# lab-cosmo/torch-pme

Hardware: AMD Instinct MI355X
Metric: atom-steps/sec (energy+forces) (higher is better)
Workload: dtype f32

## Files before the change

### torch-pme_amd/csrc/api.hip

```cpp
#include <dlfcn.h>

#include <cmath>
#include <cstring>
#include <map>
#include <string>
#include <vector>

#include "host.h"

namespace mipme {

static thread_local char g_error[512] = "";

static thread_local const char* g_last_cosched = "";
void note_cosched_kernel(const char* name) { g_last_cosched = name ? name : ""; }
static thread_local int g_last_slot_fill = 0;
void note_slot_fill(int rider_atoms) { g_last_slot_fill = rider_atoms; }
static thread_local int g_last_cell_riders = 0;
void note_cell_riders(int n) { g_last_cell_riders = n; }
void set_error(const char* fmt, ...) {
  va_list ap;
  va_start(ap, fmt);
  vsnprintf(g_error, sizeof(g_error), fmt, ap);
  va_end(ap);
// ... 97 lines not shown
  hipStream_t st = (hipStream_t)a.stream;
  const mipme_mesh_t* m = a.mesh;
  const int64_t N = a.n_atoms;
  void* bins = a.atom_bins;
  const mipme_sr_job_t* job = a.sr_job;
  int rc;
  CellWork cw{};
  if (a.out_grad_cell) cw = cell_work_layout(m, N, a.cell_work);
  const int64_t Mh = int64_t(m->nx) * m->ny * (m->nz / 2 + 1);
  double self_c, bg_c;
  correction_terms(a.pot, self_c, bg_c);
  fft_plan_begin_step(plan);
  note_slot_fill(0);
  note_cell_riders(0);
  SlotRider slots;
  struct CounterGuard {
    hipStream_t st;
    int* counters;
    size_t n;
    bool armed;
    ~CounterGuard() {
      if (armed && counters) (void)zero_async(counters, sizeof(int) * n, st);
    }
  } guard{st, nullptr, plan_counter_words(m->nx, m->ny, m->nz), false};
  if (tail && tail->slab)
    STAGE(st, "slab_moments", slab_moments_blocks<T>(st, N, (const T*)a.positions + (tail->slab - 1), 3, a.charges, 1, tail->slab_mom));
  if (bins) {
    int* counters = fft_plan_brick_count(plan);
    guard.counters = counters;
    guard.armed = true;
    const bool want_planes = !a.rho_hat && (a.flags & MIPME_FWD_RHO_MESH_UNUSED) != 0 && fft_plan_plane_forward_ok(plan);
    const bool co = job && sr_job_fusable(job);
    PlaneHost ph;
    ph.slot_values = m->n_channels == 1;
    if (want_planes) {
      ph.hat = a.hat_work;
      ph.keep_mesh = false;
    }
    const bool defer = want_planes && skip_flag_slot() == nullptr && bins_defer_slots(m, N, dtype_of<T>(), co ? job : nullptr, &ph);
    STAGE(st, "bin_atoms", bins_build<T>(st, m, N, a.positions, bins, counters, a.charges, a.out_records, want_planes, defer));
    if (defer) slots = bins_slot_rider(m, N, dtype_of<T>(), bins, a.positions, a.charges);
    {
      const int reps = (g_prof_on && co) ? kProfRepeat : 1;
      ProfScope _ps(st, co ? "spread+rspace_forward" : "spread", reps);
      bool planes = false;
      if (want_planes) {
        ph.parts = plane_spread_parts_setting();
        if (ph.parts > 1) {
          ph.hat_more = fft_plan_hat_parts(plan, st, kPlanePartsMax - 1);
          ph.more_stride = Mh * m->n_channels;
          if (!ph.hat_more) ph.parts = 1;
        }
      }
      for (int r = 0; r < reps; ++r)
        if ((rc = spread_bricks<T>(st, m, N, bins, a.charges, 1.0, a.rho_mesh, counters, co ? job : nullptr, tail != nullptr,
                                   a.out_grad_cell ? cw.cwave : nullptr, &ph, &planes))) return rc;
// ... 1309 lines not shown
```

### torch-pme_amd/csrc/bricks.hip

```cpp
#include "bricks_device.h"

namespace mipme {
bool bricks_supported(const mipme_mesh_t* m, int dtype) {
  const size_t s = dtype == MIPME_F32 ? 4 : 8;
  const int ns[3] = {m->nx, m->ny, m->nz};
  for (int d = 0; d < 3; ++d) {
    if (ns[d] <= 2 * BRICK) return false;
    const int rem = ns[d] % BRICK;
    if (rem != 0 && rem < 4) return false;
  }
  const size_t tile = BRICK + m->order - 1;
  if (2 * size_t(m->n_channels) * tile * tile * tile * s > 60 * 1024) return false;
  if (spread_stage_rows(m->order, s) == 0) return false;
  return true;
}
int64_t bins_bytes(const mipme_mesh_t* m, int64_t N, int dtype) {
  if (!bricks_supported(m, dtype)) return 0;
  return int64_t(bins_layout(m, N, dtype).total);
}
int plane_bins_capacity(const mipme_mesh_t* m, int64_t N, int dtype) { return plane_list_capacity(m, N, dtype); }
int plane_bands(const mipme_mesh_t* m, int dtype) {
  const int rows = plane_band_rows(m, dtype);
  return rows > 0 ? m->ny / rows : 0;
}
// ... 5 lines not shown
bool plane_spread_runs(const mipme_mesh_t* m, int64_t N, int dtype, const mipme_sr_job_t* job, const PlaneHost* ph, bool forward) {
  const int pcap = plane_list_capacity(m, N, dtype);
  const int band_rows = pcap > 0 ? plane_band_rows(m, dtype) : 0;
  const bool bands_ok = band_rows == m->ny || !job || (job->shift_format & kShiftFormatMask) == kShiftTable32;
  return ph && ph->hat && ph->slot_values && !ph->keep_mesh && forward && pcap > 0 && m->n_channels == 1 &&
         !sparse_bricks(N, make_brick_geom(m).nb) && !deterministic_mode() && N > 0 && band_rows > 0 && bands_ok;
}

static bool defer_slots_setting() {
  static const bool on = env_flag("MIPME_DEFER_SLOTS", true);
  return on;
}
bool bins_defer_slots(const mipme_mesh_t* m, int64_t N, int dtype, const mipme_sr_job_t* job, const PlaneHost* ph) {
  return defer_slots_setting() && N < kCoalescedBinAtoms && plane_spread_runs(m, N, dtype, job, ph, true);
}
SlotRider bins_slot_rider(const mipme_mesh_t* m, int64_t N, int dtype, void* bins, const void* pos, const void* q) {
  const BinsView v = bins_view(m, N, dtype, bins);
  SlotRider r;
  r.n_atoms = N;
  r.scheme = m->scheme;
  r.order = m->order;
  r.g = make_geom(m);
  r.pos = pos;
  r.q = q;
  r.dst = v.dst;
  r.rec = v.rec;
  r.wts = v.wts;
  r.qs = v.qs;
  r.codes = v.idx.codes;
  r.over_base = v.idx.over_base;
  return r;
}

template <typename T>
int bins_build(hipStream_t st, const mipme_mesh_t* m, int64_t n_atoms, const void* pos, void* bins, int* live,
               const void* q, void* atom_rec, bool plane_lists, bool defer_slots) {
  const int dtype = dtype_of<T>();
  const Geom g = make_geom(m);
  const BrickGeom bg = make_brick_geom(m);
  BinsView v = bins_view(m, n_atoms, dtype, bins);
  MIPME_REQUIRE(live, "the binning pass needs the live brick counters");
  if (plane_lists && v.idx.pcap > 0 && !deterministic_mode()) {
    v.idx.plive = live + bg.nb + 1;
  } else {
    v.idx.pcap = 0;
// ... 361 lines not shown
```

### torch-pme_amd/csrc/bricks_device.h

```cpp
#ifndef MIPME_BRICKS_DEVICE_H
#define MIPME_BRICKS_DEVICE_H
#include <algorithm>
#include <cmath>
#include <cstdlib>

#include <rocprim/device/device_radix_sort.hpp>

#include "host.h"
#include <map>
#include <utility>

#include "rows_body.h"
#include "fft_lds.h"

namespace mipme {

static constexpr int BRICK = 8;
static constexpr int BRICK_PTS = BRICK * BRICK * BRICK;

#define MIPME_SGPR_CAP __attribute__((amdgpu_num_sgpr(80)))
static inline int spread_stage_rows(int order, size_t real_bytes);
static inline size_t spread_row_reals(int, size_t) { return 3 * BRICK; }

struct BrickGeom {
// ... 9 lines not shown
  b.nb = b.nbx * b.nby * b.nbz;
  b.xcd = 1;
  return b;
}
static inline unsigned brick_grid(const BrickGeom& b) { return b.xcd ? pad8(unsigned(b.nb)) : unsigned(b.nb); }
__device__ __forceinline__ unsigned brick_of(const BrickGeom& b, unsigned wg) {
  return b.xcd ? xcd_contiguous(wg, unsigned(b.nb)) : wg;
}

__device__ __forceinline__ int wrap1(int a, int n) {
  a += a < 0 ? n : 0;
  return a >= n ? a - n : a;
}

struct BinsLayout {
  size_t snap, over_brick, rec, wts, codes, qs, plist, pover, wmax, epart, dst, det, det_sort_bytes, total;
  int cap;
  int pcap;
  int64_t slots;
};

static bool deterministic_mode() {
  static const bool on = env_flag("MIPME_DETERMINISTIC", false);
  return on;
}
static constexpr int kRowsPerSpreadBlock = 512 / kRowLanes;
static constexpr int kSpreadWaves = 512 / 64;

static inline int bin_capacity(int nb, int64_t N) {
  const int64_t mean = (N + nb - 1) / nb;
  int64_t cap = (4 * mean + 8 + 7) / 8 * 8;
  const int64_t all = (N + 7) / 8 * 8;
  if (cap > all) cap = all;
  return int(cap < 8 ? 8 : cap);
}

template <int N, typename T>
constexpr int wts_stride() {
  constexpr int V = 16 / int(sizeof(T));
  return (6 * N + V - 1) / V * V;
}
static inline size_t wts_stride_rt(int order, size_t elem) { return (6 * size_t(order) * elem + 15) / 16 * 16 / elem; }
// ... 61 lines not shown
  l.cap = bin_capacity(b.nb, N);
  l.slots = int64_t(b.nb) * l.cap + N;
  size_t off = 0;
  l.snap = off;       off += al(sizeof(int) * size_t(b.nb + 1));
  l.over_brick = off; off += al(sizeof(int) * size_t(N));
  l.rec = off;        off += al(sizeof(int4) * size_t(l.slots));
  l.wts = off;        off += al(wts_stride_rt(m->order, s) * s * size_t(l.slots));
  l.codes = off;      off += al(size_t(l.slots));
  l.qs = off;         off += al(s * size_t(l.slots));
  l.pcap = plane_list_capacity(m, N, dtype);
  l.plist = off;      off += al(plane_entry_bytes_rt(m->order, s) * size_t(l.pcap) * size_t(l.pcap ? m->nx * kPlaneSub : 0));
  l.pover = off;      off += al(plane_entry_bytes_rt(m->order, s) * size_t(l.pcap ? N : 0));
  l.wmax = off;       off += al(sizeof(float) * size_t(l.pcap ? (N + 63) / 64 : 0));
  l.epart = off; off += al(2 * sizeof(double) * kSpreadWaves * (((size_t(N) + kRowsPerSpreadBlock - 1) / kRowsPerSpreadBlock + 1) & ~size_t(1)));
  l.dst = off;        off += al(sizeof(int) * size_t(N));
  l.det = off;
  l.det_sort_bytes = 0;
  if (deterministic_mode()) {
    size_t sb = 0;
    unsigned* nul = nullptr;
    (void)rocprim::radix_sort_pairs(nullptr, sb, nul, nul, nul, nul, size_t(N > 0 ? N : 1), 0u, 32u, hipStream_t(0), false);
    l.det_sort_bytes = sb;
    off += 6 * al(sizeof(int) * size_t(N > 0 ? N : 1)) + al(sb);
  }
  l.total = off;
  return l;
}

struct BinIndex {
  int* live;
  int* snap;
  const int* over_brick;
  int nb, cap;
  int64_t over_base;
  unsigned char* codes = nullptr;
  int* plive = nullptr;
  int pband_shift = -1;
  void* plist = nullptr;
  void* pover = nullptr;
  int pcap = 0;
  float* wmax = nullptr;
  int n_wmax = 0;
};

template <int N>
__device__ __forceinline__ unsigned reach_code(const int (&m)[3], int nx, int ny, int nz) {
  constexpr int s0 = stencil_start<N>();
  const int n[3] = {nx, ny, nz};
  unsigned code = 0;
#pragma unroll
  for (int d = 0; d < 3; ++d) {
    const int i = m[d] & (BRICK - 1), size = min(BRICK, n[d] - (m[d] & ~(BRICK - 1)));
    code |= (i + s0 < 0 ? 1u : 0u) << (2 * d);
    code |= (i + s0 + N - 1 >= size ? 2u : 0u) << (2 * d);
  }
  return code;
}
// ... 14 lines not shown
__device__ __forceinline__ void atom_mesh_coords(const Geom& g, bool even, const T* __restrict__ pos, int64_t i,
                                                 int (&m)[3], double (&x)[3]) {
  const double rx = double(pos[3 * i + 0]), ry = double(pos[3 * i + 1]), rz = double(pos[3 * i + 2]);
  const double u[3] = {double(g.nx) * (rx * g.inv[0] + ry * g.inv[3] + rz * g.inv[6]),
                       double(g.ny) * (rx * g.inv[1] + ry * g.inv[4] + rz * g.inv[7]),
                       double(g.nz) * (rx * g.inv[2] + ry * g.inv[5] + rz * g.inv[8])};
  const int n[3] = {g.nx, g.ny, g.nz};
#pragma unroll
  for (int d = 0; d < 3; ++d) {
    int mm;
    split_runtime(u[d], even, mm, x[d]);
    m[d] = posmod(mm, n[d]);
  }
}

static constexpr int64_t kCoalescedBinAtoms = 100000;
template <int SCHEME, int N, typename T, bool COALESCE = false, bool LEAN = false>
__device__ __forceinline__ void bin_atoms_body(const Geom& g, const BrickGeom& bg, const BinIndex& bi, int64_t Natoms,
                                               const T* __restrict__ pos, int* __restrict__ over_brick,
                                               int4* __restrict__ rec, T* __restrict__ wts, const T* __restrict__ q,
                                               AtomRecord<T>* __restrict__ atom_rec, unsigned block,
                                               const int* __restrict__ slot_of = nullptr, T* __restrict__ qs = nullptr,
                                               int* __restrict__ slot_dst = nullptr) {
  static_assert(!(LEAN && COALESCE), "the lean binning pass has no weight rows to stage");
  const int64_t i = int64_t(block) * blockDim.x + threadIdx.x;
  const bool valid = i < Natoms;
  const int lane = threadIdx.x & 63;
  int b = -1;
  int m[3] = {0, 0, 0};
  double x[3] = {0.0, 0.0, 0.0};
  if (valid) {
// ... 199 lines not shown
  if (i >= r.n_atoms) return;
  const T* __restrict__ pos = static_cast<const T*>(r.pos);
  const T* __restrict__ q = static_cast<const T*>(r.q);
  const int64_t dst = r.dst[i];
  int m[3];
  double x[3];
  atom_mesh_coords<T>(r.g, (N % 2) == 0, pos, i, m, x);
  r.rec[dst] = make_int4(m[0], m[1], m[2], int(i));
  static_cast<T*>(r.qs)[dst] = q[i];
  if (dst < r.over_base) r.codes[dst] = (unsigned char)reach_code<N>(m, r.g.nx, r.g.ny, r.g.nz);
  T wx[N], wy[N], wz[N], dwx[N], dwy[N], dwz[N];
  weights_1d<SCHEME, N, true, T>(T(x[0]), wx, dwx);
  weights_1d<SCHEME, N, true, T>(T(x[1]), wy, dwy);
  weights_1d<SCHEME, N, true, T>(T(x[2]), wz, dwz);
  store_slot_weights<N, T>(static_cast<T*>(r.wts) + dst * wts_stride<N, T>(), wx, wy, wz, dwx, dwy, dwz);
}

template <typename T>
__global__ __launch_bounds__(256) void det_keys_kernel(Geom g, BrickGeom bg, bool even, int64_t Natoms, const T* __restrict__ pos,
                                                      unsigned* __restrict__ keys, unsigned* __restrict__ vals) {
  const int64_t i = int64_t(blockIdx.x) * blockDim.x + threadIdx.x;
  if (i >= Natoms) return;
  int m[3];
  double x[3];
  atom_mesh_coords<T>(g, even, pos, i, m, x);
  keys[i] = unsigned(((m[0] / BRICK) * bg.nby + m[1] / BRICK) * bg.nbz + m[2] / BRICK);
  vals[i] = unsigned(i);
}

static __global__ __launch_bounds__(256) void det_slots_kernel(int64_t Natoms, int cap, const unsigned* __restrict__ keys2,
// ... 119 lines not shown
      }                                                                                                     \
    }                                                                                                       \
  } while (0)
static __device__ long long g_wg_phase[8 * 1024];
#define MIPME_WG_PHASE(k)                                                                              \
  do {                                                                                                 \
    if (threadIdx.x == 0 && blockIdx.x < 1024) g_wg_phase[blockIdx.x * 8 + (k)] = (long long)__builtin_amdgcn_s_memrealtime(); \
  } while (0)
#else
#define MIPME_WG_STAMP(k)
#define MIPME_WG_PHASE(k)
#endif
#if defined(MIPME_WG_TIMELINE) && MIPME_WG_TIMELINE == 2
#define MIPME_WG_TIMELINE_GATHER 1
#define MIPME_WG_STAMP_GATHER(k) MIPME_WG_STAMP(k)
#else
#define MIPME_WG_TIMELINE_GATHER 0
#define MIPME_WG_STAMP_GATHER(k)
#endif

#ifndef MIPME_STAGE_SELECT
#define MIPME_STAGE_SELECT 0
#endif
#ifndef MIPME_SPREAD_UC
#define MIPME_SPREAD_UC 3
#endif
#ifndef MIPME_SPREAD_PADROWS
#define MIPME_SPREAD_PADROWS 0
#endif
#ifndef MIPME_CELL_WAVES
#define MIPME_CELL_WAVES 6
#endif
#ifndef MIPME_LIVE_PADROWS
// ... 834 lines not shown
template <int N, int NT, typename T, int THREADS = GATHER_THREADS>
__device__ __forceinline__ void load_tiles(const Geom& g, int ox, int oy, int oz, const T* __restrict__ m0,
                                           const T* __restrict__ m1, T* tile) {
  constexpr int TL = BRICK + N - 1;
  constexpr int s0 = stencil_start<N>();
  const int64_t plane = int64_t(g.ny) * g.nz;
  for (int k = threadIdx.x; k < TL * TL * TL; k += THREADS) {
    const int tx = k / (TL * TL), ty = (k / TL) % TL, tz = k % TL;
    const int gx = wrap1(ox + s0 + tx, g.nx), gy = wrap1(oy + s0 + ty, g.ny), gz = wrap1(oz + s0 + tz, g.nz);
    const int64_t gi = gx * plane + int64_t(gy) * g.nz + gz;
    tile[k] = m0[gi];
    if constexpr (NT == 2) tile[TL * TL * TL + k] = m1[gi];
  }
}

static constexpr int kGatherLanes = 8;

template <typename T>
struct GatherTail {
  const T* force;
  T force_scale;
  const T* seed;
  T* grad_pos;
  T* energy;
  const double* epart_sr;
  const double* epart_k;
  int n_sr, n_k;
  T* grad_q;
  double* rpart;
  const AtomRecord<T>* rec4;
  const T* aux_seed;
  const int* live_flags;
  double* elog = nullptr;
  int* elog_cursor = nullptr;
  int elog_cap = 0, elog_stride = 1;
  const double* slab_mom = nullptr;
  double slab_c0 = 0.0, slab_L = 0.0;
  int slab_axis = 0;
};
template <typename T>
__device__ __forceinline__ T slab_coord(const AtomRecord<T>& r, int axis) {
  return axis == 0 ? r.x : (axis == 1 ? r.y : r.z);
}
template <typename T>
static GatherTail<T> make_gather_tail(const GatherTailHost& th, const double* epart_sr, int n_sr, const void* rec4,
                                      const void* live_flags) {
  GatherTail<T> tail;
  tail.force = (const T*)th.force;
  tail.force_scale = T(th.force_scale);
  tail.seed = (const T*)th.seed;
  tail.grad_pos = (T*)th.grad_pos;
  tail.energy = (T*)th.energy;
  tail.epart_sr = epart_sr;
// ... 2 lines not shown
  tail.n_k = int(th.n_k);
  tail.grad_q = (T*)th.grad_q;
  tail.rpart = th.rpart;
  tail.rec4 = (const AtomRecord<T>*)rec4;
  tail.aux_seed = (const T*)th.aux_seed;
  tail.live_flags = (const int*)live_flags;
  tail.elog = th.elog;
  tail.elog_cursor = th.elog_cursor;
  tail.elog_cap = th.elog_cap;
  if (th.slab) {
    tail.slab_mom = th.slab_mom;
    tail.slab_c0 = th.slab_c0;
    tail.slab_L = th.slab_L;
    tail.slab_axis = th.slab - 1;
  }
  return tail;
}

template <int THREADS>
__device__ __forceinline__ void tail_rpart(double (&r3)[3], double* __restrict__ rpart, unsigned block) {
  __shared__ double rred[THREADS / 64][9];
  const int lane = threadIdx.x & 63, wave = threadIdx.x >> 6;
#pragma unroll
  for (int c = 0; c < 3; ++c) {
    double v = r3[c];
    v += __shfl_xor(v, 8, 64);
    v += __shfl_xor(v, 16, 64);
    v += __shfl_xor(v, 32, 64);
    if (lane < 3) rred[wave][3 * c + lane] = v;
  }
// ... 32 lines not shown
    double e = t[0] + 0.5 * double(inv_vol) * t[2] - 0.5 * double(self_c) * t[1] - double(bg_c) * double(inv_vol) * Q * Q;
    if constexpr (SLAB) {
      const double sQ = tail.slab_mom[0], sM = tail.slab_mom[1], sM2 = tail.slab_mom[2];
      e += 0.5 * tail.slab_c0 * (sM * sM - sQ * sM2 - sQ * sQ * tail.slab_L * tail.slab_L / 12.0);
    }
    if (tail.live_flags && (__hip_atomic_load(tail.live_flags, __ATOMIC_RELAXED, __HIP_MEMORY_SCOPE_SYSTEM) & 2)) e = __builtin_nan("");
    tail.energy[0] = T(e);
    if (tail.elog) {
      const int k = tail.elog_cursor[0];
      tail.elog[int64_t(unsigned(k) % unsigned(tail.elog_cap)) * tail.elog_stride] = double(T(e));
      tail.elog_cursor[0] = k + 1;
    }
  }
}

template <int N, bool FIELD, typename T, bool TAIL = false, int THREADS = GATHER_THREADS, bool SLAB = false>
__device__ __forceinline__ void gather_brick_body(const Geom& g, const BrickGeom& bg, int C, const BinIndex& bins,
                                                  const int4* __restrict__ rec, const T* __restrict__ wts,
                                                  const T* __restrict__ mesh, const T* __restrict__ q,
                                                  const T* __restrict__ qsum, T inv_vol, T self_c, T bg_c, bool accumulate,
                                                  T* __restrict__ out, T* __restrict__ raw, T* __restrict__ field,
                                                  unsigned block, const GatherTail<T>* tail = nullptr,
                                                  int* __restrict__ nan_flag = nullptr) {
  static_assert(N <= kGatherLanes, "one lane per z point of the stencil");
  static_assert(!TAIL || FIELD, "the tail needs the mesh field");
  static_assert(!SLAB || TAIL, "the slab term rides in the tail");
  constexpr int LANES = kGatherLanes;
  constexpr int GROUPS = THREADS / LANES;
  constexpr int TL = BRICK + N - 1;
  __shared__ T tile[TL * TL * TL];
  int bx, by, bz;
  brick_coords(bg, block, bx, by, bz);
  const int ox = bx * BRICK, oy = by * BRICK, oz = bz * BRICK;
  const int beg = int(block) * bins.cap, end = beg + bins.snap[block];
  const int n_over = bins.snap[bins.nb];
  if (bins.live && threadIdx.x == 0) {
    bins.live[block] = 0;
    if (block == 0) bins.live[bins.nb] = 0;
    if (bins.plive) {
      for (int i = int(block); i <= g.nx * kPlaneSub; i += bins.nb) bins.plive[i] = 0;
    }
  }
  T seed = T(1), seed_aux = T(1);
  if constexpr (TAIL) {
    if (tail->seed) seed = tail->seed[0];
    seed_aux = tail->aux_seed ? tail->aux_seed[0] : seed;
    if (block == 0) tail_energy<T, THREADS, SLAB>(*tail, qsum, inv_vol, self_c, bg_c);
  }
  T fA = T(0), fB = T(0), pA = T(0), pB = T(0), pK = T(0);
  if constexpr (SLAB) {
    const double sQ = tail->slab_mom[0], sM = tail->slab_mom[1], sM2 = tail->slab_mom[2], c0 = tail->slab_c0;
    fA = T(c0 * sM);
    fB = T(c0 * sQ);
    pA = T(0.5 * c0 * sM);
    pB = T(0.25 * c0 * sQ);
    pK = T(-0.5 * c0 * (0.5 * sM2 + sQ * tail->slab_L * tail->slab_L / 12.0));
  }
  double r3[3] = {0.0, 0.0, 0.0};
  if (beg == end && n_over == 0) {
    if constexpr (TAIL) {
      if (tail->rpart && threadIdx.x < 9) tail->rpart[9 * int64_t(block) + threadIdx.x] = 0.0;
    }
    return;
  }
  const int main_iters = (end - beg + GROUPS - 1) / GROUPS, over_iters = (n_over + GROUPS - 1) / GROUPS;
  const int64_t M = int64_t(g.nx) * g.ny * g.nz;
  const int l = threadIdx.x % LANES, grp = threadIdx.x / LANES;
  const bool lane_active = l < N;
  const int tz = lane_active ? l : 0;
  for (int c = 0; c < C; ++c) {
    if (c > 0) __syncthreads();
    bool staged = false;
    for (int it = 0; it < main_iters + over_iters; ++it) {
      bool valid;
      int id;
      if (it < main_iters) {
        const int idx = beg + it * GROUPS + grp;
        valid = idx < end;
        id = valid ? idx : beg;
      } else {
        const int k = (it - main_iters) * GROUPS + grp;
        valid = k < n_over && bins.over_brick[k < n_over ? k : 0] == int(block);
        id = int(bins.over_base) + (k < n_over ? k : 0);
      }
      int4 a = rec[id];
      if (!valid) a = make_int4(ox, oy, oz, 0);
      const T* wr = wts + int64_t(id) * wts_stride<N, T>();
      T wx[N], wy[N], dwx[FIELD ? N : 1], dwy[FIELD ? N : 1];
#pragma unroll
      for (int t = 0; t < N; ++t) {
        wx[t] = wr[t];
        wy[t] = wr[N + t];
        if constexpr (FIELD) {
          dwx[t] = wr[3 * N + t];
          dwy[t] = wr[4 * N + t];
        }
      }
      const T wzv = lane_active ? wr[2 * N + tz] : T(0);
      const T dwzv = (FIELD && lane_active) ? wr[5 * N + tz] : T(0);
      if (!staged) {
        load_tiles<N, 1, T, THREADS>(g, ox, oy, oz, mesh + c * M, nullptr, tile);
        staged = true;
      }
      const int64_t o_early = int64_t(a.w) * C + c;
      T q_early = T(0), out_early = T(0);
      if (q) {
        q_early = q[o_early];
        if (accumulate) out_early = out[o_early];
      }
      T f_early = T(0);
      AtomRecord<T> r_early{T(0), T(0), T(0), T(0)};
      if constexpr (TAIL) {
        f_early = tail->force[3 * int64_t(a.w) + (l < 3 ? l : 0)];
        if (SLAB || tail->rpart) r_early = tail->rec4[a.w];
      }
      if (it == 0) __syncthreads();
      const int rx = a.x - ox, ry = a.y - oy, rz = a.z - oz;
      const T* tp = tile + ry * TL + (rz + tz);
      T sA = T(0), sB = T(0), sC = T(0);
#pragma unroll
      for (int ty = 0; ty < N; ++ty) {
        T sx = T(0), sdx = T(0);
#pragma unroll
        for (int tx = 0; tx < N; ++tx) {
          const T v = tp[(rx + tx) * TL * TL + ty * TL];
          sx += v * wx[tx];
          if constexpr (FIELD) sdx += v * dwx[tx];
        }
        sA += sx * wy[ty];
        if constexpr (FIELD) {
          sB += sdx * wy[ty];
// ... 39 lines not shown
          if constexpr (SLAB) {
            const T z = slab_coord(r_early, tail->slab_axis);
            lr += z * (pA - pB * z) + pK;
          }
          const T v_final = accumulate ? out_early + lr : lr;
          out[o] = v_final;
          if constexpr (TAIL) {
            if (tail->grad_q) tail->grad_q[o] = T(2) * seed_aux * v_final;
          }
          if (nan_flag && lr != lr) *nan_flag = 1;
          if (raw) raw[o] = phi;
        } else {
          out[o] = acc;
        }
      }
    }
  }
  if constexpr (TAIL) {
    if (tail->rpart) tail_rpart<THREADS>(r3, tail->rpart, block);
  }
}

template <int N, bool FIELD, typename T>
__global__ __launch_bounds__(GATHER_THREADS) void gather_brick_kernel(Geom g, BrickGeom bg, int C, BinIndex bins,
                                                                     const int4* __restrict__ rec,
                                                                     const T* __restrict__ wts,
                                                                     const T* __restrict__ mesh, const T* __restrict__ q,
                                                                     const T* __restrict__ qsum, T inv_vol, T self_c,
                                                                     T bg_c, bool accumulate, T* __restrict__ out,
                                                                     T* __restrict__ raw, T* __restrict__ field,
// ... 5 lines not shown
}

#ifndef MIPME_GATHER_TAIL_WAVES
#define MIPME_GATHER_TAIL_WAVES 6
#endif
template <int N, typename T, int THREADS = GATHER_THREADS, bool DENSE = false, bool SLAB = false>
__global__ __launch_bounds__(THREADS, DENSE ? MIPME_GATHER_TAIL_WAVES : 1) void gather_tail_kernel(Geom g, BrickGeom bg, BinIndex bins,
                                                             const int4* __restrict__ rec, const T* __restrict__ wts,
                                                             const T* __restrict__ mesh, const T* __restrict__ q,
                                                             const T* __restrict__ qsum, T inv_vol, T self_c, T bg_c,
                                                             T* __restrict__ out, T* __restrict__ raw, T* __restrict__ field,
                                                             GatherTail<T> tail, int* __restrict__ nan_flag) {
  MIPME_WG_STAMP_GATHER(0);
  const unsigned b = brick_of(bg, blockIdx.x);
  if (b < unsigned(bg.nb))
    gather_brick_body<N, true, T, true, THREADS, SLAB>(g, bg, 1, bins, rec, wts, mesh, q, qsum, inv_vol, self_c, bg_c, true, out,
                                                       raw, field, b, &tail, nan_flag);
#if MIPME_WG_TIMELINE_GATHER
  __syncthreads();
#endif
  MIPME_WG_STAMP_GATHER(1);
}

template <int N, typename T>
__global__ __launch_bounds__(GATHER_THREADS) void gather_grad_brick_kernel(
    Geom g, BrickGeom bg, int C, BinIndex bins, const int4* __restrict__ rec, const T* __restrict__ wts,
    const T* __restrict__ q, const T* __restrict__ gout, const T* __restrict__ phi, const T* __restrict__ chi,
    const T* __restrict__ psi_dc, const T* __restrict__ gscale, T half_inv_vol, T self_c, T bg_c,
    T* __restrict__ grad_pos, T* __restrict__ grad_q, const int* __restrict__ skip) {
  static_assert(N <= kGatherLanes, "one lane per z point of the stencil");
  MIPME_SKIP_IF_SET(skip);
// ... 111 lines not shown
    }                                                                                     \
    if (!_done) {                                                                         \
      set_error("unsupported scheme/order %d/%d", int(SCHEME_V), int(ORDER_V));           \
      return MIPME_EINVAL;                                                                \
    }                                                                                     \
  } while (0)

struct BinsView {
  BinIndex idx;
  int* over_brick;
  int4* rec;
  void* wts;
  void* qs;
  double* epart;
  int* dst;
};

static inline BinsView bins_view(const mipme_mesh_t* m, int64_t N, int dtype, void* bins) {
  const BinsLayout l = bins_layout(m, N, dtype);
  const BrickGeom bg = make_brick_geom(m);
  char* b = (char*)bins;
  BinsView v;
  v.over_brick = (int*)(b + l.over_brick);
  v.idx = BinIndex{nullptr, (int*)(b + l.snap), v.over_brick, bg.nb, l.cap, int64_t(bg.nb) * l.cap};
  v.rec = (int4*)(b + l.rec);
  v.wts = (void*)(b + l.wts);
  v.idx.codes = (unsigned char*)(b + l.codes);
  v.qs = (void*)(b + l.qs);
  v.idx.pcap = l.pcap;
  if (l.pcap) {
    const int rows = plane_band_rows(m, dtype);
    if (rows > 0 && rows < m->ny) {
      int sh = 0;
      while ((kPlaneSub << sh) < m->ny) ++sh;
      v.idx.pband_shift = sh;
    }
  }
  v.idx.plist = l.pcap ? (void*)(b + l.plist) : nullptr;
  v.idx.pover = l.pcap ? (void*)(b + l.pover) : nullptr;
  v.idx.wmax = l.pcap ? (float*)(b + l.wmax) : nullptr;
  v.idx.n_wmax = l.pcap ? int((N + 63) / 64) : 0;
  v.epart = (double*)(b + l.epart);
  v.dst = (int*)(b + l.dst);
  return v;
}

}
#endif
```

### torch-pme_amd/csrc/common.h

```cpp
#pragma once

#include <hip/hip_runtime.h>
#include <cstdarg>
#include <cstdint>
#include <cstdlib>
#include <cstdio>

#include "../../include/mipme.h"

namespace mipme {

void set_error(const char* fmt, ...);
void note_cosched_kernel(const char* name);
void note_slot_fill(int rider_atoms);
void note_cell_riders(int n);

#define MIPME_CHECK_HIP(expr)                                                                 \
  do {                                                                                        \
    hipError_t _e = (expr);                                                                   \
    if (_e != hipSuccess) {                                                                   \
      mipme::set_error("%s failed: %s (%s:%d)", #expr, hipGetErrorString(_e), __FILE__, __LINE__); \
      return MIPME_EHIP;                                                                      \
    }                                                                                         \
  } while (0)
// ... 202 lines not shown
  void* energy;
  const void* epart_k;
  int64_t n_k;
  int sr_reduced;
  void* grad_q;
  double* rpart;
  const void* records;
  const void* aux_seed;
  const void* live_flags;
  double* elog;
  int* elog_cursor;
  int elog_cap;
  int slab;
  double slab_c0, slab_L;
  double* slab_mom;
};
static constexpr int kSlabBlocks = 64;
static constexpr int kSlabWork = 3 + 3 * kSlabBlocks + 1;

template <typename T>
__device__ __forceinline__ void slab_moments_body(int64_t N, const T* __restrict__ zp, int zs, const T* __restrict__ qp, int qs,
                                                  double* work, unsigned block, unsigned nblocks) {
  double acc[3] = {0.0, 0.0, 0.0};
  for (int64_t a = int64_t(block) * blockDim.x + threadIdx.x; a < N; a += int64_t(nblocks) * blockDim.x) {
    const double z = double(zp[a * zs]), q = double(qp[a * qs]);
    acc[0] += q;
    acc[1] += q * z;
    acc[2] += q * z * z;
  }
  __shared__ double red[4][3];
// ... 31 lines not shown
}

struct SlotRider {
  int64_t n_atoms = 0;
  int per_rider = 0;
  int scheme = 0, order = 0;
  Geom g;
  const void* pos = nullptr;
  const void* q = nullptr;
  const int* dst = nullptr;
  int4* rec = nullptr;
  void* wts = nullptr;
  void* qs = nullptr;
  unsigned char* codes = nullptr;
  int64_t over_base = 0;
};

struct ConvCell {
  const void* G_deriv;
  const double* cwave;
  int64_t n_waves;
  void* wbuf;
  double* rows;
  int n_riders;
  void* rho_hat_out;
  const void* rho_hat_in;
  double* kh_rows;
  int* ticket;
  const SlotRider* slots = nullptr;
};
// ... 22 lines not shown

inline const int*& skip_flag_slot() {
  static thread_local const int* p = nullptr;
  return p;
}
#define MIPME_SKIP_IF_SET(ptr)                          \
  do {                                                  \
    if ((ptr) != nullptr && *(ptr) == 1) return;        \
  } while (0)

inline bool env_flag(const char* name, bool dflt) {
  const char* e = getenv(name);
  return e ? (e[0] != '0') : dflt;
}

template <int CTRL>
__device__ __forceinline__ float dpp_mov(float v) {
  return __int_as_float(__builtin_amdgcn_update_dpp(0, __float_as_int(v), CTRL, 0xf, 0xf, true));
}
template <int CTRL>
__device__ __forceinline__ double dpp_mov(double v) {
  const int lo = __builtin_amdgcn_update_dpp(0, __double2loint(v), CTRL, 0xf, 0xf, true);
  const int hi = __builtin_amdgcn_update_dpp(0, __double2hiint(v), CTRL, 0xf, 0xf, true);
  return __hiloint2double(hi, lo);
}
__device__ __forceinline__ float read_lane(float v, int lane) {
  return __int_as_float(__builtin_amdgcn_readlane(__float_as_int(v), lane));
}
__device__ __forceinline__ double read_lane(double v, int lane) {
  return __hiloint2double(__builtin_amdgcn_readlane(__double2hiint(v), lane), __builtin_amdgcn_readlane(__double2loint(v), lane));
// ... 22 lines not shown
```

### torch-pme_amd/csrc/host.h

```cpp
#pragma once

#include <algorithm>
#include <climits>
#include <cmath>

#include "common.h"

namespace mipme {

template <typename T>
constexpr int dtype_of() {
  return sizeof(T) == 4 ? MIPME_F32 : MIPME_F64;
}

#define DT_SWITCH(dtype, CALL_F32, CALL_F64)                    \
  do {                                                          \
    if ((dtype) == MIPME_F32) return CALL_F32;                  \
    if ((dtype) == MIPME_F64) return CALL_F64;                  \
    mipme::set_error("invalid dtype %d", int(dtype));           \
    return MIPME_EINVAL;                                        \
  } while (0)

inline unsigned stride_grid(int64_t n, int block) {
  return unsigned(std::max<int64_t>(1, std::min<int64_t>((n + block - 1) / block, 2048)));
// ... 57 lines not shown
template <typename T> int pack_pair_shifts_impl(hipStream_t st, int64_t P, const void* shifts, void* packed, void* flag);
template <typename T> int distance_forward_packed_impl(hipStream_t st, int64_t P, const void* pairs, const void* packed, const void* pos,
                                                       const void* cell, void* out);
int64_t pair_partials_blocks(int64_t P);

bool bricks_supported(const mipme_mesh_t* m, int dtype);
int64_t bins_bytes(const mipme_mesh_t* m, int64_t N, int dtype);
int plane_bins_capacity(const mipme_mesh_t* m, int64_t N, int dtype);
int plane_bands(const mipme_mesh_t* m, int dtype);
const void* bins_epart(const mipme_mesh_t* m, int64_t N, int dtype, void* bins, int64_t* n);
bool sr_job_fusable(const mipme_sr_job_t* job);
template <typename T> int bins_build(hipStream_t st, const mipme_mesh_t* m, int64_t n_atoms, const void* pos, void* bins, int* live,
                                     const void* q, void* atom_rec, bool plane_lists = false, bool defer_slots = false);
bool plane_spread_runs(const mipme_mesh_t* m, int64_t N, int dtype, const mipme_sr_job_t* job, const PlaneHost* ph, bool forward);
bool bins_defer_slots(const mipme_mesh_t* m, int64_t N, int dtype, const mipme_sr_job_t* job, const PlaneHost* ph);
SlotRider bins_slot_rider(const mipme_mesh_t* m, int64_t N, int dtype, void* bins, const void* pos, const void* q);
template <typename T> int spread_bricks(hipStream_t st, const mipme_mesh_t* m, int64_t N, void* bins, const void* val, double scale, void* mesh,
                                        int* clear_count, const mipme_sr_job_t* job, bool want_epart, double* cpart, const PlaneHost* ph = nullptr,
                                        bool* used_planes = nullptr);
template <typename T> int gather_bricks(hipStream_t st, const mipme_mesh_t* m, int64_t N, void* bins, const void* mesh, const void* q,
                                        const void* qsum, double self_c, double bg_c, void* out, void* raw, int accumulate, void* field,
                                        const GatherTailHost* th, void* nan_flag, int* live);
template <typename T> int gather_grad_bricks(hipStream_t st, const mipme_mesh_t* m, int64_t N, void* bins, const void* q, const void* gout,
                                             const void* phi, const void* chi, const void* psi_dc, const void* gscale, double self_c,
                                             double bg_c, void* grad_pos, void* grad_q);

bool live_supported(const mipme_mesh_t* m, int64_t N, int dtype);
int64_t live_lists_ints(const mipme_mesh_t* m, int64_t N);
template <typename T> int live_rebin(hipStream_t st, const mipme_mesh_t* m, int64_t N, const void* rec4, void* bins, void* lists, void* host_flags);
template <typename T> int live_spread(hipStream_t st, const mipme_mesh_t* m, int64_t N, const void* rec4, void* bins, void* lists, void* mesh,
                                      const mipme_sr_job_t* job, void* host_flags, double* cpart);
// ... 107 lines not shown
```

### torch-pme_amd/ops.py

```python

from __future__ import annotations

import ctypes as C
import os
import weakref
from collections import OrderedDict

import numpy as np
import torch

from . import _front, _lib


SECOND_ORDER_HINT = (
    "torchpme_amd: the HIP kernels provide FIRST-order gradients; this graph is being differentiated twice (create_graph=True, "
    "e.g. a loss on forces).  Set `calculator.double_backward = \"analytic\"` before the forward call (the call is evaluated "
    "through differentiable primitives, exact to any order; \"auto\": only when a backward pass is itself recorded), or "
    "`calculator.double_backward = "
    "\"finite-difference\"`: the second derivative is then formed from central differences of the analytic first-order "
    "gradients (two more evaluations per double-backward pass; use float64).  Distances from `pair_distances` differentiate "
    "twice exactly either way.")


def first_order(fn, hint: str = SECOND_ORDER_HINT):
# ... 99 lines not shown
        D = torch.empty((geom.ns[0], geom.ns[1], geom.ns[2] // 2 + 1, 4), dtype=dtype, device=device)
        md = geom.desc(1)
        with _lib.on_device(device):
            _lib.check(_lib.load().mipme_kfilter_build_deriv(_lib.current_stream(device), _lib.dtype_code(dtype), C.byref(md),
                                                             C.byref(pot_desc), D.data_ptr()))
        cache.clear()
        cache[key] = D
    return D


PAIR_MODE = "rows"

TABULATE = True

MESH_MODE = "bricks"

COSCHEDULE = True
ENERGY_FAST_PATH = True
COMPACT_ENTRIES = True
FUSED_ENTRY_BYTES = 4 if COMPACT_ENTRIES else 8
TAIL_FUSION = True
SEED_PROMISE = None
TAIL_REQUEST = (False, False, None)
TAIL_LOG = None


class seed_promise:

    def __init__(self, seed, charges: bool = False, cell: bool = False, aux_seed=None, energy_log=None):
        self.seed, self.want_q, self.want_cell, self.aux_seed = seed, bool(charges), bool(cell), aux_seed
# ... 678 lines not shown
                md = geom.desc(Cn)
                plan = _lib.get_plan(device, dtype, geom.ns, Cn, geom.plan_store)
                cdtype = torch.complex64 if dtype == torch.float32 else torch.complex128
                rho_mesh = torch.empty((Cn,) + geom.ns, dtype=dtype, device=device)
                phi_mesh = torch.empty((Cn,) + geom.ns, dtype=dtype, device=device)
                rho_hat = cell_partials = None
                if not plan.xfused or not XFUSED:
                    rho_hat = torch.empty((Cn, geom.n_half), dtype=cdtype, device=device)
                hat_work = torch.empty((Cn, geom.n_half), dtype=cdtype, device=device)
                dc = torch.empty((Cn,), dtype=dtype, device=device)
                phi_atoms = torch.empty((N, Cn), dtype=dtype, device=device) if need_cell else None
                bins = None
                if MESH_MODE == "bricks":
                    nbytes = lib.mipme_atom_bins_bytes(C.byref(md), N, dt)
                    if nbytes > 0:
                        bins = torch.empty((nbytes,), dtype=torch.uint8, device=device)
                p_eff = 1 if pot_desc.kind == _lib.COULOMB else pot_desc.exponent
                slab_fusable = slab_axis is None or (Cn == 1 and p_eff == 1)
                if ENERGY_FAST_PATH and bins is not None and Cn == 1 and ctx.needs_input_grad[2] and slab_fusable:
                    field = torch.empty((N, 3), dtype=dtype, device=device)
                records_out = None
                if fused is not None and bins is not None and Cn == 1 and src_positions is positions:
                    records_out = fused["records"]
                ni = ctx.needs_input_grad
                cosched = bool(COSCHEDULE and records_out is not None and mask is None and (fused["fmt"] & 0xFF) == 1 and N > 0)
                ent32 = None
                if (cosched and fused["force"] is not None and p_eff in (1, 6) and pot_desc.smearing > 0
                        and pot_desc.exclusion_radius <= 0):
                    ent32 = topo.compact_entries(src.shifts, src.shifts_key)
                symmetric = (not full_list) or bool(topo is not None and topo.fmt_flags)
                want_q, want_cell, aux_seed = TAIL_REQUEST
# ... 901 lines not shown
```

Baseline: 601.0 million.

## Issue first gather slot loads before tile staging and batch tile loads

New measurement: 600.8 million. No clear change (-0.0%).

```diff
diff --git a/torch-pme_amd/csrc/api.hip b/torch-pme_amd/csrc/api.hip
--- a/torch-pme_amd/csrc/api.hip
+++ b/torch-pme_amd/csrc/api.hip
@@ -135,6 +135,7 @@
   note_slot_fill(0);
   note_cell_riders(0);
   SlotRider slots;
+  GatherTailHost tail_by_slot;
   struct CounterGuard {
     hipStream_t st;
     int* counters;
@@ -160,7 +161,14 @@
     }
     const bool defer = want_planes && skip_flag_slot() == nullptr && bins_defer_slots(m, N, dtype_of<T>(), co ? job : nullptr, &ph);
     STAGE(st, "bin_atoms", bins_build<T>(st, m, N, a.positions, bins, counters, a.charges, a.out_records, want_planes, defer));
-    if (defer) slots = bins_slot_rider(m, N, dtype_of<T>(), bins, a.positions, a.charges);
+    if (defer)
+      slots = bins_slot_rider(m, N, dtype_of<T>(), bins, a.positions, a.charges, tail && co ? a.out_lr : nullptr,
+                              tail && co ? tail->force : nullptr);
+    if (slots.tin) {
+      tail_by_slot = *tail;
+      tail_by_slot.slot_inputs = slots.tin;
+      tail = &tail_by_slot;
+    }
     {
       const int reps = (g_prof_on && co) ? kProfRepeat : 1;
       ProfScope _ps(st, co ? "spread+rspace_forward" : "spread", reps);
diff --git a/torch-pme_amd/csrc/bricks.hip b/torch-pme_amd/csrc/bricks.hip
--- a/torch-pme_amd/csrc/bricks.hip
+++ b/torch-pme_amd/csrc/bricks.hip
@@ -43,7 +43,8 @@
 bool bins_defer_slots(const mipme_mesh_t* m, int64_t N, int dtype, const mipme_sr_job_t* job, const PlaneHost* ph) {
   return defer_slots_setting() && N < kCoalescedBinAtoms && plane_spread_runs(m, N, dtype, job, ph, true);
 }
-SlotRider bins_slot_rider(const mipme_mesh_t* m, int64_t N, int dtype, void* bins, const void* pos, const void* q) {
+SlotRider bins_slot_rider(const mipme_mesh_t* m, int64_t N, int dtype, void* bins, const void* pos, const void* q, const void* out,
+                          const void* force) {
   const BinsView v = bins_view(m, N, dtype, bins);
   SlotRider r;
   r.n_atoms = N;
@@ -58,6 +59,11 @@
   r.qs = v.qs;
   r.codes = v.idx.codes;
   r.over_base = v.idx.over_base;
+  if (out && force && v.tin && gather_early_mode() == 2) {
+    r.tin = v.tin;
+    r.out = out;
+    r.force = force;
+  }
   return r;
 }
 
diff --git a/torch-pme_amd/csrc/bricks_device.h b/torch-pme_amd/csrc/bricks_device.h
--- a/torch-pme_amd/csrc/bricks_device.h
+++ b/torch-pme_amd/csrc/bricks_device.h
@@ -47,7 +47,8 @@
 }
 
 struct BinsLayout {
-  size_t snap, over_brick, rec, wts, codes, qs, plist, pover, wmax, epart, dst, det, det_sort_bytes, total;
+  size_t snap, over_brick, rec, wts, codes, qs, plist, pover, wmax, epart, dst, tin, det, det_sort_bytes, total;
+  bool has_tin;
   int cap;
   int pcap;
   int64_t slots;
@@ -59,6 +60,9 @@
 }
 static constexpr int kRowsPerSpreadBlock = 512 / kRowLanes;
 static constexpr int kSpreadWaves = 512 / 64;
+
+static constexpr int kSlotTailWords = 8;
+static constexpr int64_t kCoalescedBinAtoms = 100000;
 
 static inline int bin_capacity(int nb, int64_t N) {
   const int64_t mean = (N + nb - 1) / nb;
@@ -150,6 +154,8 @@
   l.wmax = off;       off += al(sizeof(float) * size_t(l.pcap ? (N + 63) / 64 : 0));
   l.epart = off; off += al(2 * sizeof(double) * kSpreadWaves * (((size_t(N) + kRowsPerSpreadBlock - 1) / kRowsPerSpreadBlock + 1) & ~size_t(1)));
   l.dst = off;        off += al(sizeof(int) * size_t(N));
+  l.has_tin = l.pcap > 0 && N < kCoalescedBinAtoms;
+  l.tin = off;        off += al(l.has_tin ? kSlotTailWords * s * size_t(l.slots) : 0);
   l.det = off;
   l.det_sort_bytes = 0;
   if (deterministic_mode()) {
@@ -177,6 +183,8 @@
   int pcap = 0;
   float* wmax = nullptr;
   int n_wmax = 0;
+  int slot_last = 0;
+  int early = 0;
 };
 
 template <int N>
@@ -221,7 +229,6 @@
   }
 }
 
-static constexpr int64_t kCoalescedBinAtoms = 100000;
 template <int SCHEME, int N, typename T, bool COALESCE = false, bool LEAN = false>
 __device__ __forceinline__ void bin_atoms_body(const Geom& g, const BrickGeom& bg, const BinIndex& bi, int64_t Natoms,
                                                const T* __restrict__ pos, int* __restrict__ over_brick,
@@ -451,6 +458,16 @@
   weights_1d<SCHEME, N, true, T>(T(x[1]), wy, dwy);
   weights_1d<SCHEME, N, true, T>(T(x[2]), wz, dwz);
   store_slot_weights<N, T>(static_cast<T*>(r.wts) + dst * wts_stride<N, T>(), wx, wy, wz, dwx, dwy, dwz);
+  if (r.tin) {
+    struct alignas(4 * sizeof(T)) Quad {
+      T e[4];
+    };
+    const T* __restrict__ out = static_cast<const T*>(r.out);
+    const T* __restrict__ force = static_cast<const T*>(r.force);
+    Quad* d = reinterpret_cast<Quad*>(static_cast<T*>(r.tin) + dst * kSlotTailWords);
+    d[0] = Quad{{pos[3 * i + 0], pos[3 * i + 1], pos[3 * i + 2], q[i]}};
+    d[1] = Quad{{out[i], force[3 * i + 0], force[3 * i + 1], force[3 * i + 2]}};
+  }
 }
 
 template <typename T>
@@ -600,9 +617,13 @@
 #if defined(MIPME_WG_TIMELINE) && MIPME_WG_TIMELINE == 2
 #define MIPME_WG_TIMELINE_GATHER 1
 #define MIPME_WG_STAMP_GATHER(k) MIPME_WG_STAMP(k)
+#define MIPME_GATHER_PHASE(k) MIPME_WG_PHASE(k)
+#define MIPME_GATHER_ARRIVED(x) asm volatile("" ::"v"(x))
 #else
 #define MIPME_WG_TIMELINE_GATHER 0
 #define MIPME_WG_STAMP_GATHER(k)
+#define MIPME_GATHER_PHASE(k)
+#define MIPME_GATHER_ARRIVED(x)
 #endif
 
 #ifndef MIPME_STAGE_SELECT
@@ -1467,6 +1488,44 @@
   }
 }
 
+static constexpr int kTileBatch = 4;
+template <int N, typename T, int THREADS>
+__device__ __forceinline__ void tile_batch_issue(const Geom& g, int ox, int oy, int oz, const T* __restrict__ m0, int k0,
+                                                 T (&v)[kTileBatch]) {
+  constexpr int TL = BRICK + N - 1, TOTAL = TL * TL * TL;
+  constexpr int s0 = stencil_start<N>();
+  const int64_t plane = int64_t(g.ny) * g.nz;
+#pragma unroll
+  for (int b = 0; b < kTileBatch; ++b) {
+    const int k = k0 + b * THREADS;
+    v[b] = T(0);
+    if (k < TOTAL) {
+      const int tx = k / (TL * TL), ty = (k / TL) % TL, tz = k % TL;
+      const int gx = wrap1(ox + s0 + tx, g.nx), gy = wrap1(oy + s0 + ty, g.ny), gz = wrap1(oz + s0 + tz, g.nz);
+      v[b] = m0[gx * plane + int64_t(gy) * g.nz + gz];
+    }
+  }
+}
+template <int N, typename T, int THREADS>
+__device__ __forceinline__ void tile_batch_commit(T* tile, int k0, const T (&v)[kTileBatch]) {
+  constexpr int TL = BRICK + N - 1, TOTAL = TL * TL * TL;
+#pragma unroll
+  for (int b = 0; b < kTileBatch; ++b) {
+    const int k = k0 + b * THREADS;
+    if (k < TOTAL) tile[k] = v[b];
+  }
+}
+template <int N, typename T, int THREADS>
+__device__ __forceinline__ void load_tile_batched(const Geom& g, int ox, int oy, int oz, const T* __restrict__ m0, T* tile,
+                                                  int k_first) {
+  constexpr int TL = BRICK + N - 1, TOTAL = TL * TL * TL;
+  for (int k0 = k_first; k0 < TOTAL; k0 += kTileBatch * THREADS) {
+    T v[kTileBatch];
+    tile_batch_issue<N, T, THREADS>(g, ox, oy, oz, m0, k0, v);
+    tile_batch_commit<N, T, THREADS>(tile, k0, v);
+  }
+}
+
 static constexpr int kGatherLanes = 8;
 
 template <typename T>
@@ -1490,6 +1549,7 @@
   const double* slab_mom = nullptr;
   double slab_c0 = 0.0, slab_L = 0.0;
   int slab_axis = 0;
+  const T* slot_in = nullptr;
 };
 template <typename T>
 __device__ __forceinline__ T slab_coord(const AtomRecord<T>& r, int axis) {
@@ -1522,6 +1582,7 @@
     tail.slab_L = th.slab_L;
     tail.slab_axis = th.slab - 1;
   }
+  tail.slot_in = (const T*)th.slot_inputs;
   return tail;
 }
 
@@ -1584,7 +1645,16 @@
   }
 }
 
-template <int N, bool FIELD, typename T, bool TAIL = false, int THREADS = GATHER_THREADS, bool SLAB = false>
+template <int N, bool FIELD, typename T>
+struct GatherSlot {
+  int4 a;
+  T wx[N], wy[N], dwx[FIELD ? N : 1], dwy[FIELD ? N : 1];
+  T wzv, dwzv;
+  T q = T(0), v = T(0), f = T(0);
+  AtomRecord<T> r{T(0), T(0), T(0), T(0)};
+};
+
+template <int N, bool FIELD, typename T, bool TAIL = false, int THREADS = GATHER_THREADS, bool SLAB = false, bool BATCH = false>
 __device__ __forceinline__ void gather_brick_body(const Geom& g, const BrickGeom& bg, int C, const BinIndex& bins,
                                                   const int4* __restrict__ rec, const T* __restrict__ wts,
                                                   const T* __restrict__ mesh, const T* __restrict__ q,
@@ -1602,8 +1672,63 @@
   int bx, by, bz;
   brick_coords(bg, block, bx, by, bz);
   const int ox = bx * BRICK, oy = by * BRICK, oz = bz * BRICK;
-  const int beg = int(block) * bins.cap, end = beg + bins.snap[block];
-  const int n_over = bins.snap[bins.nb];
+  const int64_t M = int64_t(g.nx) * g.ny * g.nz;
+  const int l = threadIdx.x % LANES, grp = threadIdx.x / LANES;
+  const bool lane_active = l < N;
+  const int tz = lane_active ? l : 0;
+  const T* __restrict__ slot_in = nullptr;
+  if constexpr (TAIL) slot_in = tail->slot_in;
+  auto issue = [&](int id, GatherSlot<N, FIELD, T>& s) __attribute__((always_inline)) {
+    s.a = rec[id];
+    const T* wr = wts + int64_t(id) * wts_stride<N, T>();
+#pragma unroll
+    for (int t = 0; t < N; ++t) {
+      s.wx[t] = wr[t];
+      s.wy[t] = wr[N + t];
+      if constexpr (FIELD) {
+        s.dwx[t] = wr[3 * N + t];
+        s.dwy[t] = wr[4 * N + t];
+      }
+    }
+    s.wzv = lane_active ? wr[2 * N + tz] : T(0);
+    s.dwzv = (FIELD && lane_active) ? wr[5 * N + tz] : T(0);
+    if constexpr (TAIL) {
+      if (slot_in) {
+        const T* ti = slot_in + int64_t(id) * kSlotTailWords;
+        if (SLAB || tail->rpart) {
+          s.r = *reinterpret_cast<const AtomRecord<T>*>(ti);
+          s.q = s.r.w;
+        } else {
+          s.q = ti[3];
+        }
+        s.v = ti[4];
+        s.f = ti[5 + (l < 3 ? l : 0)];
+      }
+    }
+  };
+  const bool early = bins.early != 0;
+  const int beg = int(block) * bins.cap;
+  const int id0 = grp <= bins.slot_last - beg ? beg + grp : bins.slot_last;
+  int cnt = 0, n_over = 0;
+  GatherSlot<N, FIELD, T> s0;
+  if (early) {
+    issue(id0, s0);
+    cnt = bins.snap[block];
+    n_over = bins.snap[bins.nb];
+    if constexpr (BATCH)
+      load_tile_batched<N, T, THREADS>(g, ox, oy, oz, mesh, tile, int(threadIdx.x));
+    else
+      load_tiles<N, 1, T, THREADS>(g, ox, oy, oz, mesh, nullptr, tile);
+    MIPME_GATHER_PHASE(2);
+    MIPME_GATHER_ARRIVED(cnt);
+    MIPME_GATHER_PHASE(1);
+  } else {
+    cnt = bins.snap[block];
+    n_over = bins.snap[bins.nb];
+    MIPME_GATHER_ARRIVED(cnt);
+    MIPME_GATHER_PHASE(1);
+  }
+  const int end = beg + cnt;
   if (bins.live && threadIdx.x == 0) {
     bins.live[block] = 0;
     if (block == 0) bins.live[bins.nb] = 0;
@@ -1627,64 +1752,50 @@
     pK = T(-0.5 * c0 * (0.5 * sM2 + sQ * tail->slab_L * tail->slab_L / 12.0));
   }
   double r3[3] = {0.0, 0.0, 0.0};
-  if (beg == end && n_over == 0) {
+  if (cnt == 0 && n_over == 0) {
     if constexpr (TAIL) {
       if (tail->rpart && threadIdx.x < 9) tail->rpart[9 * int64_t(block) + threadIdx.x] = 0.0;
     }
     return;
   }
-  const int main_iters = (end - beg + GROUPS - 1) / GROUPS, over_iters = (n_over + GROUPS - 1) / GROUPS;
-  const int64_t M = int64_t(g.nx) * g.ny * g.nz;
-  const int l = threadIdx.x % LANES, grp = threadIdx.x / LANES;
-  const bool lane_active = l < N;
-  const int tz = lane_active ? l : 0;
-  for (int c = 0; c < C; ++c) {
-    if (c > 0) __syncthreads();
-    bool staged = false;
-    for (int it = 0; it < main_iters + over_iters; ++it) {
-      bool valid;
-      int id;
-      if (it < main_iters) {
-        const int idx = beg + it * GROUPS + grp;
-        valid = idx < end;
-        id = valid ? idx : beg;
-      } else {
-        const int k = (it - main_iters) * GROUPS + grp;
-        valid = k < n_over && bins.over_brick[k < n_over ? k : 0] == int(block);
-        id = int(bins.over_base) + (k < n_over ? k : 0);
-      }
-      int4 a = rec[id];
+  const int main_iters = early ? (cnt > GROUPS ? (cnt + GROUPS - 1) / GROUPS : 1) : (cnt + GROUPS - 1) / GROUPS;
+  const int over_iters = (n_over + GROUPS - 1) / GROUPS;
+  auto finish = [&](const GatherSlot<N, FIELD, T>& s, bool valid, bool first, int c) __attribute__((always_inline)) {
+#pragma clang fp contract(on)
+      int4 a = s.a;
       if (!valid) a = make_int4(ox, oy, oz, 0);
-      const T* wr = wts + int64_t(id) * wts_stride<N, T>();
-      T wx[N], wy[N], dwx[FIELD ? N : 1], dwy[FIELD ? N : 1];
-#pragma unroll
-      for (int t = 0; t < N; ++t) {
-        wx[t] = wr[t];
-        wy[t] = wr[N + t];
-        if constexpr (FIELD) {
-          dwx[t] = wr[3 * N + t];
-          dwy[t] = wr[4 * N + t];
-        }
-      }
-      const T wzv = lane_active ? wr[2 * N + tz] : T(0);
-      const T dwzv = (FIELD && lane_active) ? wr[5 * N + tz] : T(0);
-      if (!staged) {
-        load_tiles<N, 1, T, THREADS>(g, ox, oy, oz, mesh + c * M, nullptr, tile);
-        staged = true;
-      }
+      const T(&wx)[N] = s.wx;
+      const T(&wy)[N] = s.wy;
+      const T(&dwx)[FIELD ? N : 1] = s.dwx;
+      const T(&dwy)[FIELD ? N : 1] = s.dwy;
+      const T wzv = s.wzv, dwzv = s.dwzv;
       const int64_t o_early = int64_t(a.w) * C + c;
       T q_early = T(0), out_early = T(0);
-      if (q) {
-        q_early = q[o_early];
-        if (accumulate) out_early = out[o_early];
-      }
       T f_early = T(0);
       AtomRecord<T> r_early{T(0), T(0), T(0), T(0)};
-      if constexpr (TAIL) {
-        f_early = tail->force[3 * int64_t(a.w) + (l < 3 ? l : 0)];
-        if (SLAB || tail->rpart) r_early = tail->rec4[a.w];
-      }
-      if (it == 0) __syncthreads();
+      if (TAIL && slot_in) {
+        q_early = s.q;
+        out_early = s.v;
+        f_early = s.f;
+        r_early = s.r;
+      } else {
+        if (q) {
+          q_early = q[o_early];
+          if (accumulate) out_early = out[o_early];
+        }
+        if constexpr (TAIL) {
+          f_early = tail->force[3 * int64_t(a.w) + (l < 3 ? l : 0)];
+          if (SLAB || tail->rpart) r_early = tail->rec4[a.w];
+        }
+      }
+      if (first) {
+        __syncthreads();
+        MIPME_GATHER_PHASE(3);
+        MIPME_GATHER_ARRIVED(q_early);
+        MIPME_GATHER_ARRIVED(out_early);
+        MIPME_GATHER_ARRIVED(f_early);
+        MIPME_GATHER_PHASE(4);
+      }
       const int rx = a.x - ox, ry = a.y - oy, rz = a.z - oz;
       const T* tp = tile + ry * TL + (rz + tz);
       T sA = T(0), sB = T(0), sC = T(0);
@@ -1754,6 +1865,35 @@
           out[o] = acc;
         }
       }
+      if (first) {
+        MIPME_GATHER_PHASE(5);
+      }
+  };
+  if (early) finish(s0, beg + grp < end, true, 0);
+  for (int c = 0; c < C; ++c) {
+    if (c > 0) __syncthreads();
+    for (int it = (early && c == 0) ? 1 : 0; it < main_iters + over_iters; ++it) {
+      bool valid;
+      int id;
+      if (it < main_iters) {
+        const int idx = beg + it * GROUPS + grp;
+        valid = idx < end;
+        id = valid ? idx : beg;
+      } else {
+        const int k = (it - main_iters) * GROUPS + grp;
+        valid = k < n_over && bins.over_brick[k < n_over ? k : 0] == int(block);
+        id = int(bins.over_base) + (k < n_over ? k : 0);
+      }
+      GatherSlot<N, FIELD, T> s;
+      issue(id, s);
+      if (it == 0) {
+        if (BATCH && early)
+          load_tile_batched<N, T, THREADS>(g, ox, oy, oz, mesh + c * M, tile, int(threadIdx.x));
+        else
+          load_tiles<N, 1, T, THREADS>(g, ox, oy, oz, mesh + c * M, nullptr, tile);
+        MIPME_GATHER_PHASE(2);
+      }
+      finish(s, valid, it == 0, c);
     }
   }
   if constexpr (TAIL) {
@@ -1789,7 +1929,7 @@
   MIPME_WG_STAMP_GATHER(0);
   const unsigned b = brick_of(bg, blockIdx.x);
   if (b < unsigned(bg.nb))
-    gather_brick_body<N, true, T, true, THREADS, SLAB>(g, bg, 1, bins, rec, wts, mesh, q, qsum, inv_vol, self_c, bg_c, true, out,
+    gather_brick_body<N, true, T, true, THREADS, SLAB, !DENSE>(g, bg, 1, bins, rec, wts, mesh, q, qsum, inv_vol, self_c, bg_c, true, out,
                                                        raw, field, b, &tail, nan_flag);
 #if MIPME_WG_TIMELINE_GATHER
   __syncthreads();
@@ -1931,6 +2071,7 @@
   void* qs;
   double* epart;
   int* dst;
+  void* tin;
 };
 
 static inline BinsView bins_view(const mipme_mesh_t* m, int64_t N, int dtype, void* bins) {
@@ -1959,6 +2100,9 @@
   v.idx.n_wmax = l.pcap ? int((N + 63) / 64) : 0;
   v.epart = (double*)(b + l.epart);
   v.dst = (int*)(b + l.dst);
+  v.tin = l.has_tin ? (void*)(b + l.tin) : nullptr;
+  v.idx.slot_last = int(l.slots - 1);
+  v.idx.early = gather_early_mode();
   return v;
 }
 
diff --git a/torch-pme_amd/csrc/common.h b/torch-pme_amd/csrc/common.h
--- a/torch-pme_amd/csrc/common.h
+++ b/torch-pme_amd/csrc/common.h
@@ -240,6 +240,7 @@
   int slab;
   double slab_c0, slab_L;
   double* slab_mom;
+  const void* slot_inputs;
 };
 static constexpr int kSlabBlocks = 64;
 static constexpr int kSlabWork = 3 + 3 * kSlabBlocks + 1;
@@ -301,6 +302,9 @@
   void* qs = nullptr;
   unsigned char* codes = nullptr;
   int64_t over_base = 0;
+  void* tin = nullptr;
+  const void* out = nullptr;
+  const void* force = nullptr;
 };
 
 struct ConvCell {
@@ -353,6 +357,12 @@
   return e ? (e[0] != '0') : dflt;
 }
 
+inline int gather_early_mode() {
+  const char* e = getenv("MIPME_GATHER_EARLY");
+  if (!e) return 1;
+  return e[0] == '0' ? 0 : (e[0] == '2' ? 2 : 1);
+}
+
 template <int CTRL>
 __device__ __forceinline__ float dpp_mov(float v) {
   return __int_as_float(__builtin_amdgcn_update_dpp(0, __float_as_int(v), CTRL, 0xf, 0xf, true));
diff --git a/torch-pme_amd/csrc/host.h b/torch-pme_amd/csrc/host.h
--- a/torch-pme_amd/csrc/host.h
+++ b/torch-pme_amd/csrc/host.h
@@ -95,7 +95,8 @@
                                      const void* q, void* atom_rec, bool plane_lists = false, bool defer_slots = false);
 bool plane_spread_runs(const mipme_mesh_t* m, int64_t N, int dtype, const mipme_sr_job_t* job, const PlaneHost* ph, bool forward);
 bool bins_defer_slots(const mipme_mesh_t* m, int64_t N, int dtype, const mipme_sr_job_t* job, const PlaneHost* ph);
-SlotRider bins_slot_rider(const mipme_mesh_t* m, int64_t N, int dtype, void* bins, const void* pos, const void* q);
+SlotRider bins_slot_rider(const mipme_mesh_t* m, int64_t N, int dtype, void* bins, const void* pos, const void* q,
+                          const void* out = nullptr, const void* force = nullptr);
 template <typename T> int spread_bricks(hipStream_t st, const mipme_mesh_t* m, int64_t N, void* bins, const void* val, double scale, void* mesh,
                                         int* clear_count, const mipme_sr_job_t* job, bool want_epart, double* cpart, const PlaneHost* ph = nullptr,
                                         bool* used_planes = nullptr);
diff --git a/torch-pme_amd/ops.py b/torch-pme_amd/ops.py
--- a/torch-pme_amd/ops.py
+++ b/torch-pme_amd/ops.py
@@ -137,6 +137,7 @@
 TABULATE = True
 
 MESH_MODE = "bricks"
+POISON_BINS = False
 
 COSCHEDULE = True
 ENERGY_FAST_PATH = True
@@ -845,7 +846,8 @@
                 if MESH_MODE == "bricks":
                     nbytes = lib.mipme_atom_bins_bytes(C.byref(md), N, dt)
                     if nbytes > 0:
-                        bins = torch.empty((nbytes,), dtype=torch.uint8, device=device)
+                        bins = (torch.full((nbytes,), 0xFF, dtype=torch.uint8, device=device) if POISON_BINS
+                                else torch.empty((nbytes,), dtype=torch.uint8, device=device))
                 p_eff = 1 if pot_desc.kind == _lib.COULOMB else pot_desc.exponent
                 slab_fusable = slab_axis is None or (Cn == 1 and p_eff == 1)
                 if ENERGY_FAST_PATH and bins is not None and Cn == 1 and ctx.needs_input_grad[2] and slab_fusable:
```
